# reinterpretcat/qwen3-rs

Measured on AMD Instinct MI355X. Metric: decode tokens/sec Qwen3-0.6B Q8 g=64 @1 GPU; % of int8 HBM roofline, higher is better.
Workload: dtype i8 (int8 x int8 -> i32 group dots, f32 scales/accumulate); 1 GPU; qwen3-0.6b Q8 group=64 single-stream greedy decode, 8-token prompt, reference generate-mode call pattern (first forward at pos 7, zero KV prefix), ctx 3072, 2751 tokens; mode=reference summation order (bit-identical logits), replicas=1, checkpoint_seed=1234

## Files before the change

### qwen3-rs_amd/csrc/q3_attn_short2.h

```cpp
#if defined(__HIP_DEVICE_COMPILE__) && !defined(__gfx950__)
#error "k_attn_short2 relies on gfx950 s_barrier behaviour for terminated waves; validated on gfx950 only"
#endif
constexpr int kS2Threads = 512;
constexpr int kS2MaxT = 256;
__host__ __device__ inline size_t attn_short2_smem_bytes(int hd, int max_t) { return 4 * (size_t)max_t * (size_t)(hd + 4); }

template <int V> struct IntC { static constexpr int value = V; };

#ifdef Q3_DEV
#define ATT2_STAMP(i, thr) do { if (a.stamps != nullptr && (a.debug & 64) == 0 && blockIdx.x == 3 && (int)threadIdx.x == (thr)) a.stamps[i] = __builtin_amdgcn_s_memtime(); } while (0)
#else
#define ATT2_STAMP(i, thr) do { } while (0)
#endif

template <int HD>
__global__ __launch_bounds__(kS2Threads) void k_attn_short2(const AttnArgs a) {
    static_assert(HD == 128, "head dim instantiated");
    constexpr int NQ4 = HD / 4;
    constexpr int HALF = HD / 2;
    constexpr int LD = HD + 4;
    constexpr int VT = 64;
    extern __shared__ __attribute__((aligned(16))) float ptile[];
    float* const vtile = ptile + VT * LD;
    __shared__ __attribute__((aligned(16))) float q_s[HD];
// ... 173 lines not shown
#else
        constexpr int hint = 0;
#endif
        if (hint <= 0) {
            pos = __builtin_amdgcn_readfirstlane(pos_v);
            np = pos + 1;
            if (gridDim.y == 2 && blockIdx.y == 1 && np <= 64) return;
        }
        ATT2_STAMP(8, 128);
        const int sidx = 64 * ((wave & 1) + (wave >= 6 ? 2 : 0)) + lane;
        const int r0 = sidx >> 5, col = sidx & 31;
        const unsigned loff = 4u * ((unsigned)r0 * (unsigned)kvd + 4u * (unsigned)col);
        const int kmax = max(a.seq_len / 8 - 1, 0);
        float* lp = ptile + r0 * LD + 4 * col;
        float* lv = vtile + r0 * HD + 4 * col;
        auto stage = [&](auto tier, auto with_v) {
            constexpr int T = decltype(tier)::value;
            constexpr bool V = decltype(with_v)::value != 0;
            v4f rk[T], rv[V ? T : 1];
#pragma unroll
            for (int k = 0; k < T; ++k) rk[k] = *(const v4f*)((const char*)(kbase + (size_t)min(k, kmax) * 8 * kvd) + loff);
            __builtin_amdgcn_sched_barrier(0);
            if constexpr (V) {
#pragma unroll
                for (int k = 0; k < T; ++k) rv[k] = *(const v4f*)((const char*)(vbase + (size_t)min(k, kmax) * 8 * kvd) + loff);
            }
            ATT2_STAMP(9, 128);
            if (hint > 0) {
                pos = __builtin_amdgcn_readfirstlane(pos_v);
                np = pos + 1;
            }
            __syncthreads();
            const v4f qv = ((const v4f*)q_s)[col];
#pragma unroll
            for (int k = 0; k < T; ++k) {
                const v2f p01 = (v2f){qv.x, qv.y} * (v2f){rk[k].x, rk[k].y};
                const v2f p23 = (v2f){qv.z, qv.w} * (v2f){rk[k].z, rk[k].w};
                v4f pr; pr.x = p01.x; pr.y = p01.y; pr.z = p23.x; pr.w = p23.y;
                if (r0 + 8 * k < pos) *(v4f*)(lp + 8 * k * LD) = pr;
            }
            if (wave == 7 && lane < 32) etab[lane] = etv;
            ATT2_STAMP(11, 128);
            if constexpr (V) {
                __syncthreads();
#pragma unroll
                for (int k = 0; k < T; ++k)
                    if (r0 + 8 * k < np) *(v4f*)(lv + 8 * k * HD) = rv[k];
                __builtin_amdgcn_fence(__ATOMIC_RELEASE, "workgroup");
                if (lane == 0) __hip_atomic_fetch_add(&vflag, 1u, __ATOMIC_RELAXED, __HIP_MEMORY_SCOPE_WORKGROUP);
                ATT2_STAMP(10, 128);
            }
        };
        const int tn = hint > 0 ? hint : (pos + 8) >> 3;
        if (tn <= 1) stage(IntC<1>{}, IntC<1>{});
        else if (tn <= 2) stage(IntC<2>{}, IntC<1>{});
        else if (tn <= 3) stage(IntC<3>{}, IntC<1>{});
        else if (tn <= 4) stage(IntC<4>{}, IntC<1>{});
        else if (tn <= 6) stage(IntC<6>{}, IntC<1>{});
        else if (tn <= 8) stage(IntC<8>{}, IntC<1>{});
        else if (tn <= 12) stage(IntC<12>{}, IntC<0>{});
        else if (tn <= 16) stage(IntC<16>{}, IntC<0>{});
        else if (tn <= 24) stage(IntC<24>{}, IntC<0>{});
        else stage(IntC<32>{}, IntC<0>{});
        if (np <= VT) return;
        __syncthreads();
        if (wave >= 6 || np <= 128) return;
    }
    if (wave < 2) __syncthreads();
    ATT2_STAMP(3, 0);

    const int t = 64 * wave + lane;
    float sc = -__builtin_inff();
    if (64 * wave < np) {
        const float scale = 1.0f / sqrtf((float)HD);
        const v4f* pr = (const v4f*)(ptile + min(t, pos) * LD);
        float dot = -0.0f;
        v4f pa[8], pb[8];
#pragma unroll
        for (int u = 0; u < 8; ++u) pa[u] = pr[u];
#pragma unroll
        for (int b = 0; b < NQ4 / 8; ++b) {
            if (b + 1 < NQ4 / 8) {
#pragma unroll
                for (int u = 0; u < 8; ++u) pb[u] = pr[8 * (b + 1) + u];
                __builtin_amdgcn_s_waitcnt(0xC87F);
            } else {
                __builtin_amdgcn_s_waitcnt(0xC07F);
            }
            __builtin_amdgcn_sched_barrier(0);
#pragma unroll
            for (int u = 0; u < 8; ++u) dot = chain4(dot, pa[u]);
            __builtin_amdgcn_sched_barrier(0);
#pragma unroll
            for (int u = 0; u < 8; ++u) pa[u] = pb[u];
        }
        sc = t < np ? dot * scale : -__builtin_inff();
    }
    const bool one_wave = np <= 64;
    float m;
    if (!one_wave) {
        att[t] = sc;
        if (np <= 128) {
            att[t + 128] = -__builtin_inff();
            __builtin_amdgcn_fence(__ATOMIC_RELEASE, "workgroup");
            if (lane == 0) {
                __hip_atomic_fetch_add(&bcount, 1u, __ATOMIC_RELAXED, __HIP_MEMORY_SCOPE_WORKGROUP);
                while (__hip_atomic_load(&bcount, __ATOMIC_RELAXED, __HIP_MEMORY_SCOPE_WORKGROUP) < 2u) __builtin_amdgcn_s_sleep(1);
            }
            __builtin_amdgcn_fence(__ATOMIC_ACQUIRE, "workgroup");
        } else {
            __syncthreads();
        }
        ATT2_STAMP(4, 0);
        const v4f s4 = ((const v4f*)att)[lane];
        m = fmaxf(fmaxf(s4.x, s4.y), fmaxf(s4.z, s4.w));
    } else {
// ... 15 lines not shown
```

### qwen3-rs_amd/csrc/q3_batch_host.inc

```

enum class PlanKind { Decode, Prefill, Verify, Cols, SlotPrefill };

struct BlockScratch {
    float *x = nullptr, *q = nullptr, *qn = nullptr, *kraw = nullptr, *xb = nullptr, *hb = nullptr;
    int8_t* xq_p = nullptr;
    float* xs_p = nullptr;
    State* st = nullptr;
    int* col_slot = nullptr;
    float* att_pf = nullptr;
    int att_pf_stride = 0;
    int cap = 0;
};

constexpr int kColsWidths[] = {1, 2, 4, 8, 16, 32};
constexpr int kColsNW = 6;
struct ColsPlan {
    std::vector<Launch> plan;
    Graph graph;
    size_t head = 0;
};
struct ColsHost {
    ColsCtl ctl;
    State st[kColsMax];
    int slot[kColsMax];
// ... 639 lines not shown
}

extern "C" {

int q3_batch_init(q3_engine* e, int max_streams, uint32_t ctx_len) { return batch_alloc(e, max_streams, ctx_len, true); }

int q3_prefill_batched(q3_engine* e, const int32_t* tokens, size_t n_tokens, size_t first_pos, int32_t* next_token) {
    g_err[0] = 0;
    if (!e || !tokens || n_tokens == 0) return fail(Q3_ERR_ARG, "null or empty prompt");
    if (first_pos + n_tokens > (size_t)e->cfg.seq_len)
        return fail(Q3_ERR_ARG, "first_pos %zu + n_tokens %zu exceeds seq_len %d", first_pos, n_tokens, e->cfg.seq_len);
    for (size_t i = 0; i < n_tokens; ++i)
        if (tokens[i] < 0 || tokens[i] >= e->cfg.vocab_size)
            return fail(Q3_ERR_ARG, "index out of range: token %d (vocab_size %d)", tokens[i], e->cfg.vocab_size);
    int rc;
    if (!e->batch && (rc = batch_alloc(e, kMaxStreams, 0, false, prefill_block_cap(e)))) return rc;
    BatchCtx* b = e->batch;
    HIP_TRY(hipSetDevice(e->device));
    const size_t B = (size_t)b->cap;
    if (B > (size_t)kMaxStreams) {
        const int need = (int)(((first_pos + n_tokens) + 255) & ~(size_t)255);
        if (need > b->att_pf_stride) {
            HIP_TRY(hipStreamSynchronize(e->stream));
            if (b->att_pf) (void)hipFree(b->att_pf);
            b->att_pf = nullptr;
            b->att_pf_stride = 0;
            b->plan_streams = 0;
            const size_t bytes = 4 * B * (size_t)e->cfg.n_heads * (size_t)need;
            size_t free_b = 0, total_b = 0;
            (void)hipMemGetInfo(&free_b, &total_b);
            if (bytes > free_b)
                return fail(Q3_ERR_HIP, "dense prefill: %zu MiB of score rows for blocks of %zu positions over %d positions of context do not fit "
                            "(%zu MiB free): lower Q3_PREFILL_M", bytes >> 20, B, need, free_b >> 20);
            HIP_TRY(hipMalloc((void**)&b->att_pf, bytes));
            b->att_pf_stride = need;
        }
    }
    memcpy(e->h_tokens, tokens, 4 * n_tokens);
    HIP_TRY(hipMemcpyAsync(e->d_prompt, e->h_tokens, 4 * n_tokens, hipMemcpyHostToDevice, e->stream));
    int n_last = 0;
    for (size_t base = 0; base < n_tokens; base += B) {
        const int n = (int)((n_tokens - base < B) ? n_tokens - base : B);
        n_last = n;
        if (b->plan_streams != n || b->plan_kind != PlanKind::Prefill)
            if ((rc = batch_build_plan(e, n, PlanKind::Prefill))) return rc;
        hipLaunchKernelGGL(k_set_prefill_states, dim3((n + 255) / 256), dim3(256), 0, e->stream, b->st, e->d_prompt, (int)base, (int)first_pos, n);
        for (size_t i = 0; i < b->plan_head; ++i) launch(b->plan[i], e->stream);
        HIP_TRY(hipGetLastError());
    }
    if (e->d_value_t) {
        const int kvd_ = e->cfg.n_kv_heads * e->cfg.head_dim;
        hipLaunchKernelGGL(k_value_transpose, dim3((unsigned)((kvd_ + 63) / 64), (unsigned)((n_tokens + 63) / 64), (unsigned)e->cfg.n_layers), dim3(kWG), 0,
                           e->stream, e->d_value, e->d_value_t, e->cfg.seq_len, kvd_, (int)first_pos, (int)n_tokens);
    }
    HIP_TRY(hipMemcpyAsync(e->d_x, b->x + (size_t)(n_last - 1) * e->cfg.dim, 4 * (size_t)e->cfg.dim, hipMemcpyDeviceToDevice, e->stream));
    if ((rc = e->set_state((size_t)tokens[n_tokens - 1], first_pos + n_tokens - 1))) return rc;
    for (const Launch& L : e->plan)
        if (L.fam == F_LMHEAD) launch(L, e->stream);
    HIP_TRY(hipGetLastError());
    if (e->sampling) {
        if (n_tokens > 1) hipLaunchKernelGGL(k_rng_skip, dim3(1), dim3(1), 0, e->stream, e->d_sampler, (int)(n_tokens - 1));
        if ((rc = e->enqueue_sample())) return rc;
    }
    HIP_TRY(hipMemcpyAsync(e->h_tokens, e->d_out_tokens, 4, hipMemcpyDeviceToHost, e->stream));
    HIP_TRY(hipStreamSynchronize(e->stream));
    if (next_token) *next_token = e->h_tokens[0];
    return Q3_OK;
}

int q3_forward_batch(q3_engine* e, const int32_t* tokens, const int32_t* pos, int n_streams, float* logits_out, int32_t* argmax_out) {
    g_err[0] = 0;
    if (!e) return fail(Q3_ERR_ARG, "null engine");
    int rc = batch_set_state(e, tokens, pos, n_streams);
    if (rc) return rc;
    BatchCtx* b = e->batch;
    if ((rc = batch_enqueue_step(e))) return rc;
    const size_t V = e->cfg.vocab_size;
    if (logits_out) HIP_TRY(hipMemcpyAsync(b->h_logits, b->logits, 4 * V * n_streams, hipMemcpyDeviceToHost, e->stream));
    HIP_TRY(hipMemcpyAsync(b->h_st, b->st, sizeof(State) * (size_t)n_streams, hipMemcpyDeviceToHost, e->stream));
    HIP_TRY(hipStreamSynchronize(e->stream));
    if (logits_out) memcpy(logits_out, b->h_logits, 4 * V * n_streams);
    if (argmax_out)
        for (int i = 0; i < n_streams; ++i) argmax_out[i] = b->h_st[i].token;
    return Q3_OK;
}

int q3_generate_greedy_batch(q3_engine* e, const int32_t* first_tokens, const int32_t* first_pos, int n_streams, size_t n_steps,
                             int32_t* out_tokens) {
    g_err[0] = 0;
    if (!e) return fail(Q3_ERR_ARG, "null engine");
    if (!out_tokens || n_steps == 0) return fail(Q3_ERR_ARG, "null output or zero steps");
    int rc = batch_set_state(e, first_tokens, first_pos, n_streams);
    if (rc) return rc;
    BatchCtx* b = e->batch;
    for (int i = 0; i < n_streams; ++i)
        if ((size_t)first_pos[i] + n_steps > (size_t)b->ctx)
            return fail(Q3_ERR_ARG, "stream %d: first_pos %d + n_steps %zu exceeds seq_len %d", i, first_pos[i], n_steps, b->ctx);
    for (size_t k = 0; k < n_steps; ++k)
        if ((rc = batch_enqueue_step(e))) return rc;
    for (int i = 0; i < n_streams; ++i)
        HIP_TRY(hipMemcpyAsync(b->h_tokens + (size_t)i * n_steps, b->out_tokens + (size_t)i * b->out_cap, 4 * n_steps,
                               hipMemcpyDeviceToHost, e->stream));
    HIP_TRY(hipStreamSynchronize(e->stream));
    memcpy(out_tokens, b->h_tokens, 4 * n_steps * (size_t)n_streams);
    return Q3_OK;
}
// ... 87 lines not shown
    size_t n2 = 1;
    while (n2 < (size_t)n) n2 <<= 1;
    const size_t scratch = (size_t)kSampThreads * blen;
    HIP_TRY(hipMalloc((void**)&b->spec_samp, sizeof(SamplerState) * kSpecMax));
    HIP_TRY(hipMemsetAsync(b->spec_samp, 0, sizeof(SamplerState) * kSpecMax, e->stream));
    HIP_TRY(hipMalloc((void**)&b->spec_probs, 4 * scratch * kSpecMax));
    HIP_TRY(hipMalloc((void**)&b->spec_sp, 4 * scratch * kSpecMax));
    HIP_TRY(hipMalloc((void**)&b->spec_keys, 2 * 8 * n2 * kSpecMax));
    SampleArgs a{};
    a.logits = b->logits;
    a.n = n;
    a.blen = blen;
    a.probs = b->spec_probs;
    a.keys = b->spec_keys;
    a.sp = b->spec_sp;
    a.ss = b->spec_samp;
    a.st = b->st;
    a.out_tokens = e->d_out_tokens;
    a.out_cap = 0;
    a.sb_logits = n;
    a.sb_scratch = (long long)scratch;
    a.sb_keys = 2 * (long long)n2;
    a.keys2_off = (long long)n2;
    a.pre_exp = 1;
    b->spec_sargs = a;
    return Q3_OK;
}

int spec_prepare(q3_engine* e, const char* who, bool draw = false) {
    if (e->flags & Q3_FLAG_FAST)
        return fail(Q3_ERR_UNSUPPORTED, "%s needs a reference-order engine: with Q3_FLAG_FAST the block kernels and the single-stream kernels are not bit-equal, "
                    "so a verified token need not be the token the greedy loop produces", who);
    if (e->sampling && !draw)
        return fail(Q3_ERR_UNSUPPORTED, "%s is greedy only: the engine's sampler is set to a temperature > 0 (speculative sampling is not implemented)", who);
    int rc;
    if (!e->batch && (rc = batch_alloc(e, kMaxStreams, 0, false, prefill_block_cap(e)))) return rc;
    if (e->sampling && !e->batch->spec_samp && (rc = spec_draw_alloc(e))) return rc;
    return Q3_OK;
}

int spec_pass(q3_engine* e, const int32_t* tokens, int n_real, int n_plan, size_t first_pos, float* logits_out) {
    BatchCtx* b = e->batch;
    int rc;
    HIP_TRY(hipSetDevice(e->device));
    if (b->plan_streams != n_plan || b->plan_kind != PlanKind::Verify || b->plan_draw != e->sampling)
        if ((rc = batch_build_plan(e, n_plan, PlanKind::Verify, e->sampling))) return rc;
    b->h_spec->first_pos = (int)first_pos;
    b->h_spec->n_real = n_real;
    for (int i = 0; i < kSpecMax; ++i) b->h_spec->tokens[i] = i < n_real ? tokens[i] : 0;
    HIP_TRY(hipMemcpyAsync(b->spec_io, b->h_spec, offsetof(SpecIO, n_accepted), hipMemcpyHostToDevice, e->stream));
    if ((rc = batch_enqueue_step(e))) return rc;
    HIP_TRY(hipMemcpyAsync(&b->h_spec->n_accepted, &b->spec_io->n_accepted, sizeof(SpecIO) - offsetof(SpecIO, n_accepted), hipMemcpyDeviceToHost, e->stream));
    HIP_TRY(hipStreamSynchronize(e->stream));
    if (logits_out) HIP_TRY(hipMemcpy(logits_out, b->logits, 4 * (size_t)e->cfg.vocab_size * (size_t)n_real, hipMemcpyDeviceToHost));
    return Q3_OK;
}

}

extern "C" {

}

namespace {

int verify_block(q3_engine* e, const int32_t* tokens, size_t n_tokens, size_t first_pos, int32_t* next_tokens, size_t* n_accepted, float* logits_out,
                 const char* who, bool draw) {
    g_err[0] = 0;
    if (!e || !tokens || !next_tokens || !n_accepted) return fail(Q3_ERR_ARG, "null argument");
    if (n_tokens == 0 || n_tokens > (size_t)kSpecMax) return fail(Q3_ERR_ARG, "n_tokens %zu out of range (1..%d)", n_tokens, kSpecMax);
    if (first_pos >= (size_t)e->cfg.seq_len || first_pos + n_tokens > (size_t)e->cfg.seq_len)
        return fail(Q3_ERR_ARG, "first_pos %zu + n_tokens %zu exceeds seq_len %d", first_pos, n_tokens, e->cfg.seq_len);
    for (size_t i = 0; i < n_tokens; ++i)
        if (tokens[i] < 0 || tokens[i] >= e->cfg.vocab_size)
            return fail(Q3_ERR_ARG, "index out of range: token %d (vocab_size %d)", tokens[i], e->cfg.vocab_size);
    int rc;
    if ((rc = spec_prepare(e, who, draw))) return rc;
    if ((rc = spec_pass(e, tokens, (int)n_tokens, (int)n_tokens, first_pos, logits_out))) return rc;
    const SpecIO* r = e->batch->h_spec;
    *n_accepted = (size_t)r->n_accepted;
    for (size_t i = 0; i < n_tokens; ++i) next_tokens[i] = r->next[i];
    return Q3_OK;
}

}

extern "C" {

int q3_verify(q3_engine* e, const int32_t* tokens, size_t n_tokens, size_t first_pos, int32_t* next_tokens, size_t* n_accepted, float* logits_out) {
    return verify_block(e, tokens, n_tokens, first_pos, next_tokens, n_accepted, logits_out, "q3_verify", false);
}

int q3_verify_draw(q3_engine* e, const int32_t* tokens, size_t n_tokens, size_t first_pos, int32_t* next_tokens, size_t* n_accepted, float* logits_out) {
    return verify_block(e, tokens, n_tokens, first_pos, next_tokens, n_accepted, logits_out, "q3_verify_draw", true);
}

size_t q3_lookup_draft(const int32_t* seq, size_t n, int ngram, int draft_len, int32_t* draft) {
    if (!draft) return 0;
    return lookup_draft_rescan(seq, n, ngram, draft_len, draft);
}

int q3_lookup_trace(const int32_t* seq, size_t n, size_t n_corpus, int ngram, int draft_len, int32_t* drafts, int32_t* lens) {
    g_err[0] = 0;
    if ((!seq && n) || !drafts || !lens || n_corpus > n) return fail(Q3_ERR_ARG, "null argument or n_corpus > n");
    if (ngram < 1 || draft_len < 0) return fail(Q3_ERR_ARG, "ngram %d must be >= 1 and draft_len %d >= 0", ngram, draft_len);
    LookupIndex idx(ngram);
// ... 98 lines not shown
```

### qwen3-rs_amd/csrc/q3_engine.hip

```cpp
#include <hip/hip_runtime.h>
#if !defined(__HIP_DEVICE_COMPILE__)
#include <immintrin.h>
#endif

#include <errno.h>
#include <fcntl.h>
#include <math.h>
#include <stdarg.h>
#include <stdio.h>
#include <stdlib.h>
#include <string.h>
#include <sys/mman.h>
#include <sys/stat.h>
#include <time.h>
#include <unistd.h>

#include <algorithm>
#include <map>
#include <new>
#include <string>
#include <tuple>
#include <type_traits>
#include <vector>

// ... 211 lines not shown
#define dev_knob(name, dflt) env_int(name, dflt)
#else
#define dev_knob(name, dflt) (dflt)
#endif


}

struct BatchCtx;
struct q3_engine;
namespace { void batch_free(q3_engine* e); }

struct q3_engine {
    q3_config cfg{};
    uint32_t flags = 0;
    int device = 0;
    int n_cu = 256;
    hipStream_t stream = nullptr;
    uint8_t* d_blob = nullptr;
    size_t blob_bytes = 0;
    const float *rms_att = nullptr, *rms_ffn = nullptr, *rms_final = nullptr, *q_ln = nullptr, *k_ln = nullptr;
    QT tok, wcls;
    std::vector<QT> wq, wk, wv, wo, w1, w2, w3;
    float *d_x = nullptr, *d_q = nullptr, *d_kraw = nullptr, *d_xb = nullptr, *d_hb = nullptr, *d_logits = nullptr;
    float *d_tap = nullptr, *d_key = nullptr, *d_value = nullptr, *d_rope = nullptr, *d_att = nullptr;
    float* d_value_t = nullptr;
    int8_t* d_xbq = nullptr;
    float* d_xbs = nullptr;
    State* d_state = nullptr;
    int32_t* d_out_tokens = nullptr;
    int32_t* d_prompt = nullptr;
    int out_cap = 0;
    unsigned long long* d_stamps = nullptr;
    unsigned long long* d_kacc = nullptr;
    unsigned long long* d_kslots = nullptr;
    unsigned long long* d_kcells = nullptr;
    int* d_knslots = nullptr;
    bool kstamps = false;
    unsigned long long* d_argmax_slots = nullptr;
    unsigned long long* d_next_cell = nullptr;
    int n_argmax_slots = 0;
    float* h_logits = nullptr;
    State* h_state = nullptr;
    int32_t* h_tokens = nullptr;
    std::vector<Launch> plan, plan_long;
    Launch lm_plain;
    size_t n_token_launches = 0;
    Graph decode[2], forward[2];
    float* d_att_priv = nullptr;
    int split_pos = 256;
    bool wants_value_t() const {
        return !(flags & (Q3_FLAG_FAST | Q3_FLAG_NO_VALUE_T)) && (cfg.seq_len % 4) == 0 && (int64_t)cfg.seq_len > (int64_t)split_pos &&
               dev_knob("Q3_VALUE_T", 1) != 0;
    }
    BatchCtx* batch = nullptr;
    bool sampling = false;
    SamplerState* d_sampler = nullptr;
    float* d_samp_hist = nullptr;
    int* d_samp_counts = nullptr;
    float *d_probs = nullptr, *d_sp = nullptr;
    unsigned long long* d_keys = nullptr;
    size_t keys_n2 = 0;
    std::vector<Launch> sample_plan;
    int enqueue_sample();

    int load(const char* path, uint32_t ctx_len);
    int build_plan();
    int capture();
    int enqueue_forward(size_t pos, bool draw = true);
    int set_state(size_t token, size_t pos);
    void release();
};

namespace {

struct AttnShape { AttnFn fn; dim3 grid, block; size_t smem; int kvm; };

AttnFn attn_out_fn(int slice_w, bool p_lds) {
    switch (slice_w) {
        case 8: return p_lds ? (AttnFn)k_attn_out<8, true> : (AttnFn)k_attn_out<8, false>;
        case 16: return p_lds ? (AttnFn)k_attn_out<16, true> : (AttnFn)k_attn_out<16, false>;
        case 32: return p_lds ? (AttnFn)k_attn_out<32, true> : (AttnFn)k_attn_out<32, false>;
        default: return p_lds ? (AttnFn)k_attn_out<0, true> : (AttnFn)k_attn_out<0, false>;
    }
}
AttnFn attn_scores_fn(int kvm) { return kvm == 4 ? (AttnFn)k_attn_scores_kv<4> : kvm == 2 ? (AttnFn)k_attn_scores_kv<2> : (AttnFn)k_attn_scores; }

AttnShape attn_scores_shape(int hd, int n_heads, int n_kv_heads, int S) {
    const int kv_mul = n_heads / n_kv_heads;
    AttnShape r;
    r.kvm = (hd != kSgHd || (kv_mul != 2 && kv_mul != 4) || !dev_knob("Q3_ATT_SCORES_KV", 1)) ? 0 : kv_mul;
    const int tch = r.kvm == 4 ? sg_tch<4>() : r.kvm == 2 ? sg_tch<2>() : attn_tch(hd);
    r.fn = attn_scores_fn(r.kvm);
    r.grid = dim3((unsigned)(r.kvm ? n_kv_heads : n_heads), (unsigned)((S + tch - 1) / tch));
    r.block = dim3(kWG);
    r.smem = r.kvm == 4 ? attn_scores_kv_smem_bytes<4>() : r.kvm == 2 ? attn_scores_kv_smem_bytes<2>() : attn_scores_smem_bytes(hd);
    return r;
}
AttnShape attn_out_shape(int hd, int n_heads, int S, int slice_w) {
    return AttnShape{attn_out_fn(slice_w, attn_out_p_in_lds(S)), dim3((unsigned)n_heads, (unsigned)(hd / slice_w)), dim3(kAoThreads),
                     attn_out_smem_bytes(hd, S, slice_w), 0};
}
AttnShape attn_short_shape(int hd, int n_heads, int S) {
    if (hd == 128 && S >= 8 && (S % 8) == 0)
        return AttnShape{(AttnFn)k_attn_short2<128>, dim3((unsigned)n_heads, 2), dim3(kS2Threads), attn_short2_smem_bytes(128, kS2MaxT), 0};
    return AttnShape{hd == 128 ? (AttnFn)k_attn_short<128> : (AttnFn)k_attn_short<64>, dim3((unsigned)n_heads), dim3(kWG), 0, 0};
// ... 305 lines not shown
    }
#endif

    auto base_args = [&](int n) {
        GemvArgs a{};
        a.n = n;
        a.group = G;
        a.strict = strict;
        a.debug = kstamps ? 64 : 0;
        a.st = d_state;
        a.seq_len = S;
        return a;
    };
    int rc;
    auto stamp_cells = [&]() -> unsigned long long* {
        if (!d_stamps) return nullptr;
        return kstamps ? d_kslots + 2 * (size_t)kKstampSlots * plan.size() : d_stamps + 16 * plan.size();
    };
    auto stamp = [&](GemvArgs& a) {
        if (d_stamps) { a.stamps = stamp_cells(); a.stamp_block = dev_knob("Q3_STAMP_BLOCK", 7); }
    };
    auto gemv = [&](Launch& Ln, Family fam, GemvArgs a, int pro, int epi, int n, int units, int qkv_hd, bool stamped) -> int {
        GemvLaunch g;
        if ((rc = plan_role(g, a, pro, epi, n, units, G, fast_fold, qkv_hd, n_cu))) return rc;
        if (stamped) stamp(a);
        return make_launch(Ln, fam, g.fn, dim3(g.grid), dim3(g.block), g.smem, a);
    };
    auto push_both = [&](const Launch& Ln) { plan.push_back(Ln); plan_long.push_back(Ln); };
    HIP_TRY(hipMalloc((void**)&d_xbq, (size_t)ahd));
    HIP_TRY(hipMalloc((void**)&d_xbs, 4 * (size_t)(ahd / G)));
    Launch Ln;
    for (int l = 0; l < L; ++l) {
        const size_t kv_off = (size_t)l * S * kvd;
        {
            GemvArgs a = base_args(dim);
            a.seg[0] = Seg{wq[l].q, wq[l].s, d_q, ahd, 0};
            a.seg[1] = Seg{wk[l].q, wk[l].s, d_kraw, kvd, 0};
            a.seg[2] = Seg{wv[l].q, wv[l].s, d_value + kv_off, kvd, kvd};
            a.v_t = d_value_t ? d_value_t + kv_off : nullptr;
            a.total_rows = ahd + 2 * kvd;
            for (int k = 0; k < 2; ++k) {
                a.qkv_dw[k] = (const char*)a.seg[k + 1].wq - (const char*)a.seg[k].wq;
                a.qkv_ds[k] = (const char*)a.seg[k + 1].ws - (const char*)a.seg[k].ws;
                a.qkv_do[k] = (const char*)a.seg[k + 1].out - (const char*)a.seg[k].out;
            }
            a.norm_w = rms_att + (size_t)l * dim;
            a.in = d_x;
            if (l == 0) {
                a.emb_q = tok.q;
                a.emb_s = tok.s;
                a.x_out = d_x;
            }
            if ((rc = gemv(Ln, F_QKV, a, l == 0 ? PRO_EMBED_NORM : PRO_NORM, EPI_QKV, dim, a.total_rows, hd, true))) return rc;
            push_both(Ln);
        }
        const bool att_short = (hd == 64 || hd == 128) && split_pos <= kShortMaxT && dev_knob("Q3_ATT_SHORT", 1);
        const GemvCfg* wo_preq = att_short ? find_cfg(PRO_PREQR, EPI_RESID, ahd, G, fast_fold) : nullptr;
        {
            AttnArgs a{};
            a.q = d_q;
            a.key_cache = d_key + kv_off;
            a.k_raw = d_kraw;
            a.value_cache = d_value + kv_off;
            a.value_t = d_value_t ? d_value_t + kv_off : nullptr;
            a.q_norm_w = q_ln + (size_t)l * hd;
            a.k_norm_w = k_ln + (size_t)l * hd;
            a.rope = d_rope;
            a.xb = d_xb;
            a.att_global = use_att_global ? d_att : nullptr;
            a.st = d_state;
            a.pos_override = -1;
            attn_set_heads(a, cfg.n_heads, cfg.n_kv_heads);
            a.hd = hd;
            a.seq_len = S;
            a.strict = strict;
            a.write_q = 0;
            a.debug = kstamps ? 64 : 0;
            a.stamps = stamp_cells();
            if (wo_preq) {
                a.xbq = d_xbq;
                a.xbs = d_xbs;
                a.xb_group = G;
            }
            Launch A, B;
            if ((rc = make_split_attn(A, B, a, d_att, d_att + (size_t)cfg.n_heads * att_stride, d_att_priv, n_cu))) return rc;
            plan_long.push_back(A);
            plan_long.push_back(B);
            if (att_short) {
                const AttnShape sh = attn_short_shape(hd, cfg.n_heads, S);
                rc = make_launch(Ln, F_ATTN, sh.fn, sh.grid, sh.block, sh.smem, a);
            } else {
                rc = make_launch(Ln, F_ATTN, k_attn, dim3((unsigned)cfg.n_heads), dim3(kWG), attn_smem_bytes(hd, use_att_global ? 0 : S), a);
            }
            if (rc) return rc;
            plan.push_back(Ln);
        }
        {
            GemvArgs a = base_args(ahd);
            a.seg[0] = Seg{wo[l].q, wo[l].s, d_x, dim, 0};
            a.total_rows = dim;
            a.in = d_xb;
            a.pre_q = d_xbq;
            a.pre_s = d_xbs;
            if ((rc = gemv(Ln, F_WO, a, PRO_QUANT, EPI_RESID, ahd, dim, 1, false))) return rc;
            plan_long.push_back(Ln);
            if ((rc = gemv(Ln, F_WO, a, wo_preq ? PRO_PREQR : PRO_QUANT, EPI_RESID, ahd, dim, 1, true))) return rc;
            plan.push_back(Ln);
// ... 32 lines not shown
        a.argmax_slots = d_argmax_slots;
        stamp(a);
        HIP_TRY(hipMalloc((void**)&d_next_cell, 16));
        HIP_TRY(hipMemset(d_next_cell, 0, 16));
        a.next_cell = d_next_cell;
        a.out_tokens = d_out_tokens;
        a.out_cap = out_cap;
        a.prompt = d_prompt;
        if ((rc = make_launch(Ln, F_LMHEAD, g.fn, dim3(g.grid), dim3(g.block), g.smem, a))) return rc;
        push_both(Ln);
        a.next_cell = nullptr;
        if ((rc = make_launch(lm_plain, F_LMHEAD, g.fn, dim3(g.grid), dim3(g.block), g.smem, a))) return rc;
    }
    n_token_launches = plan.size();
#ifdef Q3_DEV
    if (kstamps) {
        const int nl = (int)n_token_launches;
        std::vector<int> ns(plan.size(), 0);
        for (size_t i = 0; i < plan.size(); ++i) {
            const long w = (long)plan[i].grid.x * plan[i].grid.y * (plan[i].block.x / 64);
            ns[i] = (int)(w < kKstampSlots ? w : kKstampSlots);
        }
        HIP_TRY(hipMemcpy(d_knslots, ns.data(), 4 * ns.size(), hipMemcpyHostToDevice));
        if ((rc = make_launch(Ln, F_NEXT, k_kstamp_reduce, dim3((unsigned)nl), dim3(256), 0, d_kslots, d_knslots, d_kcells))) return rc;
        push_both(Ln);
        if ((rc = make_launch(Ln, F_NEXT, k_kstamp_fold, dim3(1), dim3(256), 0, d_kcells, nl, d_kacc))) return rc;
        push_both(Ln);
    }
#endif
    return Q3_OK;
}

int q3_engine::capture() {
    const size_t lbytes = 4 * (size_t)cfg.vocab_size;
    const bool fwd = dev_knob("Q3_FWD_GRAPH", 1) != 0;
    for (int lng = 0; lng < 2; ++lng) {
        const std::vector<Launch>& P = lng ? plan_long : plan;
        int rc = decode[lng].capture(stream, [&] {
            for (const Launch& L : P) launch(L, stream);
            return Q3_OK;
        });
        if (rc == Q3_OK && fwd)
            rc = forward[lng].capture(stream, [&]() -> int {
                HIP_TRY(hipMemcpyAsync(d_state, h_state, sizeof(State), hipMemcpyHostToDevice, stream));
                for (const Launch& L : P) launch(L, stream);
                HIP_TRY(hipMemcpyAsync(h_logits, d_logits, lbytes, hipMemcpyDeviceToHost, stream));
                return Q3_OK;
            });
        if (rc) return rc;
    }
    return Q3_OK;
}

int q3_engine::enqueue_forward(size_t pos, bool draw) {
    const int lng = (int64_t)pos >= (int64_t)split_pos ? 1 : 0;
    if (decode[lng]) {
        int rc = decode[lng].launch(stream);
        if (rc) return rc;
    } else {
        for (const Launch& L : (lng ? plan_long : plan)) launch(L, stream);
        HIP_TRY(hipGetLastError());
    }
    return draw ? enqueue_sample() : Q3_OK;
}

int q3_engine::enqueue_sample() {
    if (!sampling) return Q3_OK;
    for (const Launch& L : sample_plan) launch(L, stream);
    HIP_TRY(hipGetLastError());
    return Q3_OK;
}

int q3_engine::set_state(size_t token, size_t pos) {
    if (token >= (size_t)cfg.vocab_size || pos >= (size_t)cfg.seq_len)
        return fail(Q3_ERR_ARG, "index out of range: token %zu (vocab_size %d), pos %zu (seq_len %d)", token,
                    cfg.vocab_size, pos, cfg.seq_len);
    h_state->token = (int)token;
    h_state->pos = (int)pos;
    h_state->step = 0;
    h_state->prompt_len = 0;
    h_state->argmax = 0ull;
    HIP_TRY(hipMemcpyAsync(d_state, h_state, sizeof(State), hipMemcpyHostToDevice, stream));
    return Q3_OK;
}

extern "C" {

const char* q3_last_error(void) { return g_err; }
uint32_t q3_abi_version(void) { return Q3_ABI_VERSION; }

int q3_parse_header(const uint8_t* data, size_t len, q3_config* out) {
    g_err[0] = 0;
    return parse_header(data, len, out);
}

int q3_create(const char* checkpoint_path, uint32_t ctx_len, int device, uint32_t flags, q3_engine** out) {
    g_err[0] = 0;
    if (!checkpoint_path || !out) return fail(Q3_ERR_ARG, "null argument");
    *out = nullptr;
    int ndev = 0;
    if (hipGetDeviceCount(&ndev) != hipSuccess || ndev <= 0)
        return fail(Q3_ERR_HIP, "no HIP device available (libqwen3_hip has no CPU fallback)");
    if (device < 0 || device >= ndev) return fail(Q3_ERR_ARG, "device %d out of range (%d devices)", device, ndev);
    q3_engine* e = new q3_engine();
    e->flags = flags;
    e->device = device;
    int rc = e->load(checkpoint_path, ctx_len);
    if (rc == Q3_OK) rc = e->build_plan();
    if (rc == Q3_OK && !(flags & Q3_FLAG_NO_GRAPH)) rc = e->capture();
    if (rc != Q3_OK) {
        e->release();
        delete e;
        return rc;
    }
    *out = e;
    return Q3_OK;
}

void q3_destroy(q3_engine* e) {
    if (!e) return;
    (void)hipSetDevice(e->device);
    if (e->stream) (void)hipStreamSynchronize(e->stream);
    e->release();
    delete e;
}

int q3_get_config(const q3_engine* e, q3_config* out) {
    if (!e || !out) return fail(Q3_ERR_ARG, "null argument");
    *out = e->cfg;
    return Q3_OK;
}

const float* q3_forward(q3_engine* e, size_t token, size_t pos) {
    g_err[0] = 0;
    if (!e) {
        fail(Q3_ERR_ARG, "null engine");
        return nullptr;
    }
    static const bool dbg = getenv("Q3_DEBUG_TIMING") != nullptr;
    struct timespec t0, t1, t2, t3, t4;
    if (dbg) clock_gettime(CLOCK_MONOTONIC, &t0);
    if (hipSetDevice(e->device) != hipSuccess) { fail(Q3_ERR_HIP, "hipSetDevice failed"); return nullptr; }
    const int lng = (int64_t)pos >= (int64_t)e->split_pos ? 1 : 0;
    if (e->forward[lng] && !e->sampling) {
        if (token >= (size_t)e->cfg.vocab_size || pos >= (size_t)e->cfg.seq_len) {
            fail(Q3_ERR_ARG, "index out of range: token %zu (vocab_size %d), pos %zu (seq_len %d)", token, e->cfg.vocab_size, pos, e->cfg.seq_len);
            return nullptr;
        }
        e->h_state->token = (int)token;
        e->h_state->pos = (int)pos;
        e->h_state->step = 0;
        e->h_state->prompt_len = 0;
        e->h_state->argmax = 0ull;
        hipError_t ge = hipGraphLaunch(e->forward[lng].exec, e->stream);
        if (ge == hipSuccess) ge = hipStreamSynchronize(e->stream);
        if (ge != hipSuccess) {
            fail(Q3_ERR_HIP, "forward failed: %s", hipGetErrorString(ge));
            return nullptr;
        }
        return e->h_logits;
    }
    if (e->set_state(token, pos) != Q3_OK) return nullptr;
    if (dbg) clock_gettime(CLOCK_MONOTONIC, &t1);
    if (e->enqueue_forward(pos, false) != Q3_OK) return nullptr;
    if (dbg) clock_gettime(CLOCK_MONOTONIC, &t2);
    hipError_t err = hipMemcpyAsync(e->h_logits, e->d_logits, 4 * (size_t)e->cfg.vocab_size, hipMemcpyDeviceToHost, e->stream);
    if (dbg) clock_gettime(CLOCK_MONOTONIC, &t3);
    if (err == hipSuccess) err = hipStreamSynchronize(e->stream);
    if (err != hipSuccess) {
        fail(Q3_ERR_HIP, "forward failed: %s", hipGetErrorString(err));
        return nullptr;
    }
    if (dbg) {
        clock_gettime(CLOCK_MONOTONIC, &t4);
        auto us = [](const timespec& a, const timespec& b) { return (b.tv_sec - a.tv_sec) * 1e6 + (b.tv_nsec - a.tv_nsec) * 1e-3; };
        static int n = 0;
        if (++n % 16 == 0)
            fprintf(stderr, "[q3] forward: set_state %.1f us, graph launch %.1f us, D2H enqueue %.1f us, sync %.1f us\n",
                    us(t0, t1), us(t1, t2), us(t2, t3), us(t3, t4));
    }
    return e->h_logits;
}

int q3_forward_argmax(q3_engine* e, size_t token, size_t pos, int32_t* next_token) {
    g_err[0] = 0;
    if (!e || !next_token) return fail(Q3_ERR_ARG, "null argument");
    HIP_TRY(hipSetDevice(e->device));
    int rc = e->set_state(token, pos);
    if (rc) return rc;
    if ((rc = e->enqueue_forward(pos))) return rc;
    HIP_TRY(hipMemcpyAsync(e->h_tokens, e->d_out_tokens, 4, hipMemcpyDeviceToHost, e->stream));
    HIP_TRY(hipStreamSynchronize(e->stream));
    *next_token = e->h_tokens[0];
    return Q3_OK;
}

int q3_generate_greedy(q3_engine* e, size_t first_token, size_t first_pos, size_t n_tokens, int32_t* out_tokens) {
    g_err[0] = 0;
    if (!e || (!out_tokens && n_tokens)) return fail(Q3_ERR_ARG, "null argument");
    if (n_tokens == 0) return Q3_OK;
    if (first_pos + n_tokens > (size_t)e->cfg.seq_len)
        return fail(Q3_ERR_ARG, "first_pos %zu + n_tokens %zu exceeds seq_len %d", first_pos, n_tokens, e->cfg.seq_len);
    HIP_TRY(hipSetDevice(e->device));
    int rc = e->set_state(first_token, first_pos);
    if (rc) return rc;
    struct timespec t0, t1, t2;
// ... 123 lines not shown
    a.st = e->d_state;
    a.out_tokens = e->d_out_tokens;
    a.out_cap = e->out_cap;
    a.pre_exp = dev_knob("Q3_SAMPLER_PRE_EXP", 1);
    a.phase = (a.pre_exp && dev_knob("Q3_SAMPLER_PIPELINE", 1)) ? 1 : 0;
    a.hist = e->d_samp_hist;
    a.counts = e->d_samp_counts;
    a.stamps = e->d_stamps ? e->d_stamps + 16 * (size_t)(5 * e->cfg.n_layers + 3) : nullptr;
    e->sample_plan.clear();
    int rc = Q3_OK;
    auto add = [&](void (*k)(const SampleArgs), dim3 grid, dim3 block, size_t smem, const SampleArgs& sa) {
        Launch L;
        if (rc == Q3_OK && (rc = make_launch(L, F_NEXT, k, grid, block, smem, sa)) == Q3_OK) e->sample_plan.push_back(L);
    };
    if (a.pre_exp) add(k_sample_exp, dim3((unsigned)e->n_cu, 1), dim3(256), 0, a);
    add(k_sample, dim3(1), dim3(kSampThreads), 4 * kSegFloats, a);
    if (a.phase == 1) {
        SampleArgs tail = a;
        tail.phase = 2;
        add(k_sample_norm_hist, dim3(kSampGrid), dim3(256), 0, a);
        add(k_sample_count, dim3(kSampGrid), dim3(256), 0, a);
        add(k_sample_scatter, dim3(kSampGrid), dim3(256), 0, a);
        add(k_sample, dim3(1), dim3(kSampThreads), 4 * kSegFloats, tail);
    }
    if (rc) return rc;
    e->sampling = temperature != 0.0f;
    return Q3_OK;
}

int q3_sampler_get_rng(q3_engine* e, uint64_t* rng_state) {
    g_err[0] = 0;
    if (!e || !rng_state || !e->d_sampler) return fail(Q3_ERR_ARG, "q3_sampler_set has not been called");
    HIP_TRY(hipSetDevice(e->device));
    HIP_TRY(hipStreamSynchronize(e->stream));
    SamplerState h;
    HIP_TRY(hipMemcpy(&h, e->d_sampler, sizeof(h), hipMemcpyDeviceToHost));
    *rng_state = h.rng;
    return Q3_OK;
}

int q3_forward_sample(q3_engine* e, size_t token, size_t pos, int32_t* next_token) { return q3_forward_argmax(e, token, pos, next_token); }

int q3_generate_sampled(q3_engine* e, size_t first_token, size_t first_pos, size_t n_tokens, int32_t* out_tokens) {
    return q3_generate_greedy(e, first_token, first_pos, n_tokens, out_tokens);
}

int q3_reset_kv(q3_engine* e) {
    if (!e) return fail(Q3_ERR_ARG, "null engine");
    HIP_TRY(hipSetDevice(e->device));
    const size_t bytes = 4 * (size_t)e->cfg.n_layers * e->cfg.seq_len * e->cfg.n_kv_heads * e->cfg.head_dim;
    HIP_TRY(hipMemsetAsync(e->d_key, 0, bytes, e->stream));
    HIP_TRY(hipMemsetAsync(e->d_value, 0, bytes, e->stream));
    if (e->d_value_t) HIP_TRY(hipMemsetAsync(e->d_value_t, 0, bytes, e->stream));
    HIP_TRY(hipMemsetAsync(e->d_next_cell, 0, 16, e->stream));
    HIP_TRY(hipStreamSynchronize(e->stream));
    return Q3_OK;
}

int q3_read_state(q3_engine* e, int kind, size_t offset, size_t count, float* out) {
    if (!e || !out) return fail(Q3_ERR_ARG, "null argument");
    HIP_TRY(hipSetDevice(e->device));
    const size_t kv = (size_t)e->cfg.n_layers * e->cfg.seq_len * e->cfg.n_kv_heads * e->cfg.head_dim;
    const float* src = nullptr;
    size_t lim = 0;
    if (kind == 0) { src = e->d_key; lim = kv; }
    else if (kind == 1) { src = e->d_value; lim = kv; }
    else if (kind == 2) { src = e->d_tap; lim = (size_t)e->cfg.dim; }
    else return fail(Q3_ERR_ARG, "unknown state kind %d", kind);
    if (offset + count > lim) return fail(Q3_ERR_ARG, "state range out of bounds");
    HIP_TRY(hipStreamSynchronize(e->stream));
    HIP_TRY(hipMemcpy(out, src + offset, 4 * count, hipMemcpyDeviceToHost));
    return Q3_OK;
}

const char* q3_profile_name(int family) { return (family >= 0 && family < F_COUNT) ? kFamilyNames[family] : nullptr; }

int q3_profile(q3_engine* e, size_t token, size_t pos, int reps, float* ms, int32_t* launches, int cap) {
    g_err[0] = 0;
    if (!e || !ms || !launches || cap < F_COUNT || reps <= 0) return fail(Q3_ERR_ARG, "bad argument");
    HIP_TRY(hipSetDevice(e->device));
    for (int i = 0; i < cap; ++i) { ms[i] = 0.f; launches[i] = 0; }
    const std::vector<Launch>& P = ((int64_t)pos >= (int64_t)e->split_pos) ? e->plan_long : e->plan;
    const size_t nl = P.size();
    struct Events {
        std::vector<hipEvent_t> ev;
        ~Events() { for (hipEvent_t x : ev) if (x) (void)hipEventDestroy(x); }
    } evs;
    evs.ev.assign(2 * F_COUNT, nullptr);
    std::vector<hipEvent_t>& ev = evs.ev;
    for (auto& x : ev) HIP_TRY(hipEventCreate(&x));
    for (int r = 0; r < reps; ++r) {
        int rc = e->set_state(token, pos);
        if (rc) return rc;
        auto replay = [&](const Launch& L) { launch(L.fam == F_LMHEAD ? e->lm_plain : L, e->stream); };
        for (size_t i = 0; i < nl; ++i) replay(P[i]);
        for (int f = 0; f < F_COUNT; ++f) {
            HIP_TRY(hipEventRecord(ev[2 * f], e->stream));
            for (size_t i = 0; i < nl; ++i)
                if (P[i].fam == f) { replay(P[i]); launches[f] += 1; }
            HIP_TRY(hipEventRecord(ev[2 * f + 1], e->stream));
        }
        HIP_TRY(hipStreamSynchronize(e->stream));
        for (int f = 0; f < F_COUNT; ++f) {
            float t = 0.f;
            HIP_TRY(hipEventElapsedTime(&t, ev[2 * f], ev[2 * f + 1]));
            ms[f] += t;
        }
    }
    return F_COUNT;
}

}

namespace {
#if !defined(__HIP_DEVICE_COMPILE__)
__attribute__((target("avx2"))) size_t copy_argmax_last_avx2(const float* src, float* dst, size_t n) {
    const __m256i m7f = _mm256_set1_epi32(0x7fffffff);
    __m256i best = _mm256_set1_epi32(INT32_MIN), bidx = _mm256_setzero_si256();
    __m256i cur = _mm256_setr_epi32(0, 1, 2, 3, 4, 5, 6, 7);
    const __m256i step = _mm256_set1_epi32(8);
    size_t i = 0;
    for (; i + 8 <= n; i += 8) {
        const __m256i b = _mm256_loadu_si256((const __m256i*)(src + i));
        _mm256_stream_si256((__m256i*)(dst + i), b);
        const __m256i key = _mm256_xor_si256(b, _mm256_and_si256(_mm256_srai_epi32(b, 31), m7f));
        const __m256i lt = _mm256_cmpgt_epi32(best, key);
        best = _mm256_max_epi32(best, key);
        bidx = _mm256_blendv_epi8(cur, bidx, lt);
        cur = _mm256_add_epi32(cur, step);
    }
    _mm_sfence();
    alignas(32) int32_t kk[8], ii[8];
    _mm256_store_si256((__m256i*)kk, best);
    _mm256_store_si256((__m256i*)ii, bidx);
    int32_t best_key = INT32_MIN;
    size_t best_i = 0;
    for (int l = 0; l < 8; ++l)
        if (kk[l] > best_key || (kk[l] == best_key && (size_t)ii[l] > best_i)) { best_key = kk[l]; best_i = (size_t)ii[l]; }
    for (; i < n; ++i) {
        int32_t b;
        memcpy(&b, src + i, 4);
        dst[i] = src[i];
        const int32_t key = b ^ ((b >> 31) & 0x7fffffff);
        if (key >= best_key) { best_key = key; best_i = i; }
    }
    return best_i;
// ... 513 lines not shown
```

Baseline: 1132 tokens/s.

## Defer transposed-V mirror writes to long-context plan and specialize short-attn tiers

The short-context decode plan no longer writes the transposed value cache in its QKV epilogue (v_t set to null). Instead, a host-tracked row counter triggers a batched k_value_transpose catch-up when decode crosses into the long plan. Prefill and speculative paths update the counter. The short attention kernel also dispatches through a switch with finer-grained template tiers, so fewer unused tile rows are processed. The cost is extra host-side state and a one-off transpose launch at the split point, and a stale counter would risk incorrect V_t contents.

```diff
diff --git a/qwen3-rs_amd/csrc/q3_attn_short2.h b/qwen3-rs_amd/csrc/q3_attn_short2.h
--- a/qwen3-rs_amd/csrc/q3_attn_short2.h
+++ b/qwen3-rs_amd/csrc/q3_attn_short2.h
@@ -249,16 +249,17 @@
             }
         };
         const int tn = hint > 0 ? hint : (pos + 8) >> 3;
-        if (tn <= 1) stage(IntC<1>{}, IntC<1>{});
-        else if (tn <= 2) stage(IntC<2>{}, IntC<1>{});
-        else if (tn <= 3) stage(IntC<3>{}, IntC<1>{});
-        else if (tn <= 4) stage(IntC<4>{}, IntC<1>{});
-        else if (tn <= 6) stage(IntC<6>{}, IntC<1>{});
-        else if (tn <= 8) stage(IntC<8>{}, IntC<1>{});
-        else if (tn <= 12) stage(IntC<12>{}, IntC<0>{});
-        else if (tn <= 16) stage(IntC<16>{}, IntC<0>{});
-        else if (tn <= 24) stage(IntC<24>{}, IntC<0>{});
-        else stage(IntC<32>{}, IntC<0>{});
+#define S2_TIER(T, V) case T: stage(IntC<T>{}, IntC<V>{}); break
+#define S2_TIER2(T) case T - 1: case T: stage(IntC<T>{}, IntC<0>{}); break
+        switch (tn) {
+            case 0:
+            S2_TIER(1, 1); S2_TIER(2, 1); S2_TIER(3, 1); S2_TIER(4, 1); S2_TIER(5, 1); S2_TIER(6, 1); S2_TIER(7, 1); S2_TIER(8, 1);
+            S2_TIER(9, 0); S2_TIER(10, 0); S2_TIER(11, 0); S2_TIER(12, 0); S2_TIER(13, 0); S2_TIER(14, 0); S2_TIER(15, 0); S2_TIER(16, 0);
+            S2_TIER2(18); S2_TIER2(20); S2_TIER2(22); S2_TIER2(24); S2_TIER2(26); S2_TIER2(28); S2_TIER2(30);
+            default: stage(IntC<32>{}, IntC<0>{}); break;
+        }
+#undef S2_TIER
+#undef S2_TIER2
         if (np <= VT) return;
         __syncthreads();
         if (wave >= 6 || np <= 128) return;
diff --git a/qwen3-rs_amd/csrc/q3_batch_host.inc b/qwen3-rs_amd/csrc/q3_batch_host.inc
--- a/qwen3-rs_amd/csrc/q3_batch_host.inc
+++ b/qwen3-rs_amd/csrc/q3_batch_host.inc
@@ -715,6 +715,7 @@
         const int kvd_ = e->cfg.n_kv_heads * e->cfg.head_dim;
         hipLaunchKernelGGL(k_value_transpose, dim3((unsigned)((kvd_ + 63) / 64), (unsigned)((n_tokens + 63) / 64), (unsigned)e->cfg.n_layers), dim3(kWG), 0,
                            e->stream, e->d_value, e->d_value_t, e->cfg.seq_len, kvd_, (int)first_pos, (int)n_tokens);
+        e->value_t_mirrored(first_pos, n_tokens);
     }
     HIP_TRY(hipMemcpyAsync(e->d_x, b->x + (size_t)(n_last - 1) * e->cfg.dim, 4 * (size_t)e->cfg.dim, hipMemcpyDeviceToDevice, e->stream));
     if ((rc = e->set_state((size_t)tokens[n_tokens - 1], first_pos + n_tokens - 1))) return rc;
@@ -908,6 +909,7 @@
     if ((rc = batch_enqueue_step(e))) return rc;
     HIP_TRY(hipMemcpyAsync(&b->h_spec->n_accepted, &b->spec_io->n_accepted, sizeof(SpecIO) - offsetof(SpecIO, n_accepted), hipMemcpyDeviceToHost, e->stream));
     HIP_TRY(hipStreamSynchronize(e->stream));
+    e->value_t_mirrored(first_pos, (size_t)b->h_spec->n_accepted + 1);
     if (logits_out) HIP_TRY(hipMemcpy(logits_out, b->logits, 4 * (size_t)e->cfg.vocab_size * (size_t)n_real, hipMemcpyDeviceToHost));
     return Q3_OK;
 }
diff --git a/qwen3-rs_amd/csrc/q3_engine.hip b/qwen3-rs_amd/csrc/q3_engine.hip
--- a/qwen3-rs_amd/csrc/q3_engine.hip
+++ b/qwen3-rs_amd/csrc/q3_engine.hip
@@ -287,6 +287,11 @@
     bool wants_value_t() const {
         return !(flags & (Q3_FLAG_FAST | Q3_FLAG_NO_VALUE_T)) && (cfg.seq_len % 4) == 0 && (int64_t)cfg.seq_len > (int64_t)split_pos &&
                dev_knob("Q3_VALUE_T", 1) != 0;
+    }
+    int vt_rows = 0;
+    int value_t_before(size_t pos);
+    void value_t_mirrored(size_t first, size_t n) {
+        if (d_value_t && (size_t)vt_rows >= first && (size_t)vt_rows < first + n) vt_rows = (int)(first + n);
     }
     BatchCtx* batch = nullptr;
     bool sampling = false;
@@ -698,7 +703,10 @@
                 a.x_out = d_x;
             }
             if ((rc = gemv(Ln, F_QKV, a, l == 0 ? PRO_EMBED_NORM : PRO_NORM, EPI_QKV, dim, a.total_rows, hd, true))) return rc;
-            push_both(Ln);
+            plan_long.push_back(Ln);
+            a.v_t = nullptr;
+            if ((rc = gemv(Ln, F_QKV, a, l == 0 ? PRO_EMBED_NORM : PRO_NORM, EPI_QKV, dim, a.total_rows, hd, true))) return rc;
+            plan.push_back(Ln);
         }
         const bool att_short = (hd == 64 || hd == 128) && split_pos <= kShortMaxT && dev_knob("Q3_ATT_SHORT", 1);
         const GemvCfg* wo_preq = att_short ? find_cfg(PRO_PREQR, EPI_RESID, ahd, G, fast_fold) : nullptr;
@@ -837,8 +845,25 @@
     return Q3_OK;
 }
 
+int q3_engine::value_t_before(size_t pos) {
+    if (!d_value_t) return Q3_OK;
+    if ((int64_t)pos < (int64_t)split_pos) {
+        if ((size_t)vt_rows > pos) vt_rows = (int)pos;
+        return Q3_OK;
+    }
+    if ((size_t)vt_rows < pos) {
+        const int kvd = cfg.n_kv_heads * cfg.head_dim, n = (int)pos - vt_rows;
+        hipLaunchKernelGGL(k_value_transpose, dim3((unsigned)((kvd + 63) / 64), (unsigned)((n + 63) / 64), (unsigned)cfg.n_layers), dim3(kWG), 0, stream,
+                           (const float*)d_value, d_value_t, cfg.seq_len, kvd, vt_rows, n);
+        HIP_TRY(hipGetLastError());
+    }
+    if ((size_t)vt_rows < pos + 1) vt_rows = (int)pos + 1;
+    return Q3_OK;
+}
+
 int q3_engine::enqueue_forward(size_t pos, bool draw) {
     const int lng = (int64_t)pos >= (int64_t)split_pos ? 1 : 0;
+    if (int rc = value_t_before(pos)) return rc;
     if (decode[lng]) {
         int rc = decode[lng].launch(stream);
         if (rc) return rc;
@@ -937,6 +962,7 @@
         e->h_state->step = 0;
         e->h_state->prompt_len = 0;
         e->h_state->argmax = 0ull;
+        if (e->value_t_before(pos) != Q3_OK) return nullptr;
         hipError_t ge = hipGraphLaunch(e->forward[lng].exec, e->stream);
         if (ge == hipSuccess) ge = hipStreamSynchronize(e->stream);
         if (ge != hipSuccess) {
@@ -1166,6 +1192,7 @@
     HIP_TRY(hipMemsetAsync(e->d_key, 0, bytes, e->stream));
     HIP_TRY(hipMemsetAsync(e->d_value, 0, bytes, e->stream));
     if (e->d_value_t) HIP_TRY(hipMemsetAsync(e->d_value_t, 0, bytes, e->stream));
+    e->vt_rows = 0;
     HIP_TRY(hipMemsetAsync(e->d_next_cell, 0, 16, e->stream));
     HIP_TRY(hipStreamSynchronize(e->stream));
     return Q3_OK;
@@ -1206,6 +1233,7 @@
     for (int r = 0; r < reps; ++r) {
         int rc = e->set_state(token, pos);
         if (rc) return rc;
+        if ((rc = e->value_t_before(pos))) return rc;
         auto replay = [&](const Launch& L) { launch(L.fam == F_LMHEAD ? e->lm_plain : L, e->stream); };
         for (size_t i = 0; i < nl; ++i) replay(P[i]);
         for (int f = 0; f < F_COUNT; ++f) {
```

Result: no change. 1129 tokens/s (-0.2%).
